# vikshiv/mumemto

Hardware: AMD Instinct MI355X
Metric: input Gbp/s end-to-end (higher is better)
Workload: dtype u8 text, u32 (+u8 beyond 2^32) positions, u32 LCP

## Files before the change

### __graft_entry__.py

```python
import os
import sys

ROOT = os.path.dirname(os.path.abspath(__file__))
for p in (ROOT, os.path.join(ROOT, "oracle")):
    if p not in sys.path:
        sys.path.insert(0, p)


def build():
    import subprocess
    from mumemto_amd import build as mbuild
    lib = mbuild.build(verbose=True)
    assert os.path.exists(lib)
    subprocess.check_call(["make", "-C", os.path.join(ROOT, "oracle"), "all"])
    subprocess.check_call(["make", "-C", os.path.join(ROOT, "tests", "fake_rccl")])
    subprocess.check_call(["make", "-C", os.path.join(ROOT, "tests", "corrupt_rccl")])
    subprocess.check_call(["make", "-C", os.path.join(ROOT, "tests", "kprobe")])
    subprocess.check_call(["make", "-C", os.path.join(ROOT, "tests", "kprobe_input")])
    import mumemto_amd
    mumemto_amd.load_library()


def smoke():
    import numpy as np
    import mumemto_amd
    import pyoracle as O
    from mumemto_amd import synth

    docs = synth.pangenome(6, 50000, 0.01, seed=4, inversion=(2, 10000, 14000))
    eng = mumemto_amd.Engine(0)
    eng.set_docs(docs)
    eng.run(merge_metadata=True)
    want = O.run(docs, merge=True)
# ... 17 lines not shown
```

### mumemto_amd/csrc/engine.hpp

```cpp
#pragma once
#include <cstdint>
#include <cstring>
#include <functional>
#include <memory>
#include <string>
#include <vector>

#include "../../include/mumemto_gpu.h"
#include "device_utils.hpp"
#include "kernels.hpp"
#include "merge_types.hpp"
#include "pfp.hpp"
#include "piece_writer.hpp"
#include "sorter.hpp"
#include "textref.hpp"

namespace mmt {

struct HostRows {
    bool mum_mode = true;
    size_t n_docs = 0, n_rows = 0, n_occ = 0;
    const uint32_t* length = nullptr;
    const int64_t* mum_offsets = nullptr;
    const uint8_t* mum_strands = nullptr;
// ... 172 lines not shown
    void pfp_prepare(uint32_t w, uint32_t p);
    void pfp_prepare_emitter(uint32_t w);
    void pfp_group_tables(uint32_t E, uint32_t G, uint64_t out_lo, uint64_t out_hi, bool slim);
    void pfp_emit_codes(int shift);
    void guided_prepare();
    void guided_check_errors(const char* what);
    void build_giant(const std::vector<uint64_t>& hist);
    static int symbol_codes(const std::vector<uint64_t>& hist, int lowest, bool dollar, uint8_t code[256]);
    struct RunEnds { DevBuf<uint32_t> ends, sorted, count; };
    struct DictLcpScratch { DevBuf<uint32_t> plcp, counts, huge; };
    int sort_dictionary(const uint8_t* dict, uint32_t nd, const std::vector<uint64_t>& hist, DevBuf<uint8_t>& code, uint32_t reserve,
                        int chars_cap, DevBuf<uint32_t>& sa, DevBuf<uint32_t>& rank, RunEnds* run_list);
    void dictionary_lcp(const uint8_t* dict, uint32_t nd, uint32_t* sa, const uint32_t* esuf, const uint8_t* ebw,
                        DevBuf<uint32_t>& lcp, DictLcpScratch& X, uint32_t cap, const char* whose);
    void sort_parse();
    void build_inverted_lists(bool rec12, bool drop_other_form, uint32_t pos_bits, uint32_t* k_in, uint32_t* v_in);
    void pfp_stream(ScanState& S, const mmt_params& p);
    void pfp_emit_window(uint64_t b0, uint64_t c1, int set);
    uint64_t pfp_first_tile(uint64_t b0);
    void guided_stream(ScanState& S, const mmt_params& p);
    void guided_stream_expand(ScanState& S, const mmt_params& p);
    void lcp_bwt();
    void scan(const mmt_params& p);
    void scan_begin(const mmt_params& p, ScanState& S);
    bool scan_window(ScanState& S, const ColWindow& w, const mmt_params& p);
    void scan_end(ScanState& S);
    void window_reserve(int set, uint64_t entries);
    ColWindow window_view(int set, uint64_t base, uint32_t len, uint32_t first) const;
    bool hand_off_window(ScanState& S, int set, const ColWindow& w, const mmt_params& p, bool closing_entry);
    void shard_range(uint32_t index, uint64_t& lo, uint64_t& hi) const;
    struct GuidedShare { std::vector<uint64_t> pre; uint32_t bin_lo = 0, bin_hi = 0; };
// ... 119 lines not shown
```

### mumemto_amd/csrc/pfp.cpp

```cpp
#include <algorithm>
#include <chrono>
#include <cstdio>
#include <cstdlib>
#include <stdexcept>

#include "engine.hpp"
#include "pfp_kernels.hpp"
#include "pool.hpp"
#include "prims.hpp"

namespace mmt {

static void offsets_from_counts(DevBuf<uint8_t>& temp, const uint32_t* counts, PosBuf& out, size_t n, hipStream_t s) {
    if (out.wide()) prims::exclusive_sum_u32_to_u64(temp, counts, out.p64(), n, s);
    else prims::exclusive_sum_u32(temp, counts, out.p32(), n, s);
}


int Engine::symbol_codes(const std::vector<uint64_t>& hist, int lowest, bool dollar, uint8_t code[256]) {
    int sigma = 0;
    for (int c = 0; c < 256; c++) code[c] = (c >= lowest && (hist[c] || (dollar && c == 2))) ? (uint8_t)(++sigma) : 0;
    return sigma;
}

// ... 58 lines not shown
    MMT_HIP(hipStreamSynchronize(st));
}

void Engine::sort_parse() {
    PfpState& S = *pfp_;
    hipStream_t st = stream_;
    const uint32_t m = S.n_phrases;
    S.sa_p.ensure(m); S.isa_p.ensure(m);
    const int pbits = bit_width_u64((uint64_t)S.n_distinct);
    const int pchars = std::max(1, 64 / pbits);
    sorter_.reserve(m);
    pk::pack_keys_u32(S.parse.get(), m, pbits, pchars, sorter_.keys_in(), sorter_.vals_in(), st);
    S.rounds_parse = sorter_.sort(m, pbits * pchars, (uint64_t)pchars, S.sa_p.get(), S.isa_p.get(), d_temp_, st);
}

void Engine::build_inverted_lists(bool rec12, bool drop_other_form, uint32_t pos_bits, uint32_t* k_in, uint32_t* v_in) {
    PfpState& S = *pfp_;
    const bool W = wide_;
    hipStream_t st = stream_;
    const uint32_t m = S.n_phrases, D = S.n_distinct;
    pk::occ_sequence(S.sa_p.get(), S.pid.get(), m, D, k_in, v_in, st);
    prims::sort_pairs_u32_u32(d_temp_, k_in, S.occ_ids.get(), v_in, S.occ_ts.get(), (size_t)m + 1, 0, bit_width_u64((uint64_t)D), st);
    if (rec12) {
        if (drop_other_form) { S.occ.release(); S.occ_sl.release(); }
        S.occ12.ensure(3 * (size_t)m + 4);
        pk::occ_finish12(S.occ_ids.get(), S.occ_ts.get(), S.sa_p.get(), S.pstart.get(), W, m, S.occ_start.get(),
                         S.occ12.get(), S.plcp.sl.get(), st);
    } else {
        if (drop_other_form) S.occ12.release();
        S.occ.ensure(m); S.occ_sl.ensure(m);
        pk::occ_finish(S.occ_ids.get(), S.occ_ts.get(), S.sa_p.get(), S.pstart.get(), m, S.occ_start.get(), S.occ.get(),
                       pos_bits, S.plcp.sl.get(), S.occ_sl.get(), W, st);
    }
    MMT_HIP(hipStreamSynchronize(st));
}

void Engine::pfp_parse(uint32_t w, uint32_t p, bool keep_dict_inputs) {
    PfpState& S = *pfp_;
    const uint64_t n = n_;
    const bool W = wide_;
    const bool slim = (lean_ || wide_) && !keep_dict_inputs;
    if (w < 1 || w > 32 || p < 1) throw std::runtime_error("PFP window must be in [1, 32] and the modulus positive");
    std::vector<uint64_t> hist;
    d2h(hist, d_hist_.get(), 256, stream_);
// ... 178 lines not shown
    const uint32_t m = S.n_phrases, D = S.n_distinct;
    EventPair e5, e6;
    e5.start(st);
    sort_parse();
    if (slim) { MMT_HIP(hipStreamSynchronize(st)); sorter_.release(); S.isa_p.release(); S.parse.release(); }
    S.plcp.build(text_ref(), n + 1 + w, S.sa_p.get(), S.pid.get(), S.pstart.get(), W, m, d_temp_, st);
    e5.stop(st);
    mem_mark(device_, "parse suffix array + LCP");

    e6.start(st);
    const int shift = bit_width_u64((uint64_t)m + 1);
    const uint32_t nd = S.dict_len;
    const uint32_t pos_bits = W ? (uint32_t)bit_width_u64(n + w + 1) : 32u;
    if ((uint32_t)shift + pos_bits > 64)
        throw std::runtime_error("parse rank and text position do not fit one 64-bit occurrence record");
    S.occ_start.ensure((size_t)D + 2); S.occ.ensure(m);
    S.occ_ids.ensure((size_t)m + 1); S.occ_ts.ensure((size_t)m + 1);
    {
        DevBuf<uint32_t> k_own, v_own;
        uint32_t *k_in, *v_in;
        if (slim) { k_own.ensure((size_t)m + 1); v_own.ensure((size_t)m + 1); k_in = k_own.get(); v_in = v_own.get(); }
        else {
            sorter_.u32_a().ensure((size_t)m + 1); sorter_.u32_b().ensure((size_t)m + 1);
            k_in = sorter_.u32_a().get(); v_in = sorter_.u32_b().get();
        }
        build_inverted_lists(false, false, pos_bits, k_in, v_in);
    }
    if (slim) { S.occ_ids.release(); S.occ_ts.release(); S.sa_p.release(); S.pid.release(); S.pstart.release(); }
    S.vscan.ensure(nd); S.ptab.ensure((size_t)D * 16 + 16);
    prims::exclusive_sum_u32(d_temp_, S.vflag.get(), S.vscan.get(), nd, st);
    const uint32_t E = S.n_entries = read_u32(S.vscan.get() + (nd - 1), st) + read_u32(S.vflag.get() + (nd - 1), st);
    pk::phrase_table(S.occ_start.get(), S.plen.get(), S.rep.get(), D, S.ptab.get(), st);
    S.ce_cnt.ensure(E); S.ce_eoff.ensure(E, W); S.ce_first.ensure(E); S.ce_offm1.ensure(E); S.ce_gs.ensure(E);
    S.ce_bwt.ensure(E); S.ce_hl.ensure(E); S.ce_slen.ensure(E);
    if (!S.gscan.get() || !S.segmin.get()) throw std::runtime_error("PFP tables released too early");
    pk::entry_compact(S.esuf.get(), S.ephr.get(), S.ebw.get(), S.gflag.get(), S.gscan.get(), S.vflag.get(), S.vscan.get(),
                      S.segmin.get(), S.ptab.get(), nd, S.ce_cnt.get(), S.ce_first.get(), S.ce_offm1.get(), S.ce_bwt.get(),
                      S.ce_gs.get(), S.ce_hl.get(), S.ce_slen.get(), st);
    offsets_from_counts(d_temp_, S.ce_cnt.get(), S.ce_eoff, E, st);
    {
        const uint64_t total = S.ce_eoff.read(E - 1, st) + read_u32(S.ce_cnt.get() + (E - 1), st);
        if (total != n + 1) throw std::runtime_error("PFP expansion does not cover the text exactly once");
    }
    if (slim) {
        S.esuf.release(); S.ephr.release(); S.ebw.release(); S.gflag.release(); S.vflag.release(); S.vscan.release();
        S.ptab.release(); S.plen.release(); S.segmin.release();
    }
    S.occ12.release(); S.emit_pos_bits = pos_bits; S.emit_w = w;
    pfp_emit_codes(shift);
    pfp_group_tables(E, S.n_groups, 0, n + 1, slim);
    S.emit_launches = 0;
    S.emit_ready = true;
    S.bwt_ready = true;
    e6.stop(st);
    mem_mark(device_, "lists + emitter tables");
    S.ms[5] = e5.ms(); S.ms[6] = e6.ms();
    sort_rounds_ = S.rounds_dict;
}

void Engine::pfp_group_tables(uint32_t E, uint32_t G, uint64_t out_lo, uint64_t out_hi, bool slim) {
    PfpState& S = *pfp_;
    const bool W = wide_;
    hipStream_t st = stream_;
// ... 50 lines not shown
    MMT_HIP(hipStreamSynchronize(st));
    if (slim) S.gscan.release();

    S.tiles = (out_hi + TILE - 1) / TILE;
    S.tile_base = out_lo / TILE;
    pk::EmitArgs& ea = S.ea;
    ea = pk::EmitArgs();
    ea.wide = W;
    ea.segb = S.segb.get(); ea.sege = S.sege.get(); ea.n_groups = G;
    ea.ce_eoff = S.ce_eoff.get(); ea.ce_cnt = S.ce_cnt.get(); ea.ce_first = S.ce_first.get();
    ea.ce_offm1 = S.ce_offm1.get(); ea.ce_bwt = S.ce_bwt.get(); ea.ce_gs = S.ce_gs.get();
    ea.n = n_;
    ea.fb_group = S.fb_group.get(); ea.fb_off = S.fb_off.get(); ea.n_fb = F; ea.fb_base = 0;
    ea.err = S.err.get();
    ea.ghead = S.ghead.get();
    ea.occ = S.occ.get(); ea.occ_sl = S.occ_sl.get(); ea.occ12 = S.occ12.get(); ea.pos_bits = S.emit_pos_bits;
    ea.rmq = S.plcp.view(); ea.w = S.emit_w;
    ea.bwt_code = S.bwt_code.get(); ea.fb_bits = S.fb_bits;
    S.tile_first.ensure((size_t)(S.tiles - S.tile_base) + 4);
    pk::tile_first(S.segb.get(), G, S.tiles, S.tile_first.get(), W, st, S.tile_base);
    MMT_HIP(hipMemsetAsync(S.err.get(), 0, 64, st));
}

void Engine::pfp_emit_codes(int shift) {
    PfpState& S = *pfp_;
    hipStream_t st = stream_;
    S.decode = pk::BwtDecode{};
    S.fb_bits = 0; S.key_shift = shift;
    if (!sw::on(sw::MMT_PFP_NO_BWT_CODE)) {
        std::vector<uint64_t> hist;
        d2h(hist, d_hist_.get(), 256, st);
// ... 164 lines not shown
```

### mumemto_amd/csrc/pfp.hpp

```cpp
#pragma once
#include <unordered_map>
#include <cstdint>
#include <vector>

#include "device_utils.hpp"
#include "parse_lcp.hpp"
#include "guided_kernels.hpp"
#include "pfp_kernels.hpp"

namespace mmt {

struct PfpSummary {
    uint32_t w = 0, p = 0;
    uint32_t n_cuts = 0, n_phrases = 0, n_distinct = 0, dict_len = 0, n_groups = 0;
    bool guided = false;
    bool expand = false;
    int rounds_dict = 0, rounds_parse = 0;
    uint64_t run_refined = 0;
    float ms[8] = {0};
    uint32_t n_entries = 0, n_fallback = 0, emit_launches = 0;
    bool bwt_ready = false;
    int g_prefix = 0;
    uint32_t g_share_lo = 0, g_share_hi = 0;
    int g_bits = 0;
// ... 3 lines not shown

struct PfpState : PfpSummary {
    bool have_parse = false;
    DevBuf<uint8_t> dict, ptab, pinfo;
    DevBuf<uint16_t> tmask;
    DevBuf<uint32_t> tcnt, toff;
    PosBuf cuts, pstart;
    DevBuf<uint32_t> plen, iota, ord_a, order, scan, dflags, pid, rep, dlen, dstart, esuf, ephr;
    DevBuf<uint64_t> dinfo;
    DevBuf<uint8_t> ebw;
    DevBuf<uint32_t> sa_d, rank_d, gflag, pflag, gscan, pscan, prank, parse, sa_p, isa_p, err;
    DevBuf<uint64_t> h1, h2, hk_a, hk_b;
    DevBuf<uint32_t> occ_start, occ_ids, occ_ts, vflag, vscan;
    DevBuf<uint64_t> occ;
    DevBuf<uint32_t> occ12;
    uint32_t emit_pos_bits = 0, emit_w = 0;
    DevBuf<uint32_t> ce_cnt, ce_first, ce_offm1, ce_gs, sege, xk_a, xk_b, fb_group, fb_size, fb_rel, tile_first;
    DevBuf<uint8_t> emit_plan;
    PosBuf ce_eoff, segb, fb_off, fb_start, xv_a, xv_b;
    DevBuf<uint8_t> ce_bwt, bwt_code;
    ParseLcp plcp;
    DevBuf<uint32_t> ghead, ce_hl, ce_slen, occ_sl, lcp_d;
    DevBuf<uint64_t> segmin;
    std::unordered_map<uint64_t, uint64_t> first_tile;
    bool emit_ready = false;
    pk::EmitArgs ea;
    pk::BwtDecode decode{};
    uint32_t fb_bits = 0;
    int key_shift = 0;
    uint64_t tiles = 0, tile_base = 0;
// ... 16 lines not shown
```

### mumemto_amd/csrc/pfp_kernels.hip

```cpp
#include <hip/hip_runtime.h>

#include <algorithm>
#include <cstddef>
#include <cstdint>
#include <cstdlib>
#include <string>

#include "device_utils.hpp"
#include "kernels.hpp"
#include "launch_grid.hpp"
#include "pfp_kernels.hpp"

namespace mmt { namespace pk {

template <int BLOCK>
__global__ __launch_bounds__(BLOCK) void k_trigger_masks(const TextRef T, uint64_t n, uint32_t w,
                                                         uint32_t p, uint32_t pot,
                                                         uint16_t* __restrict__ masks,
                                                         uint32_t* __restrict__ block_count, uint32_t block0) {
    constexpr int PER = 16;
    __shared__ uint32_t s_cnt;
    if (threadIdx.x == 0) s_cnt = 0;
    __syncthreads();
    const uint64_t blk = (uint64_t)blockIdx.x + block0;
// ... 607 lines not shown
__global__ void k_occ_sequence(const uint32_t* __restrict__ sa_p, const uint32_t* __restrict__ pid, uint32_t m,
                               uint32_t D, uint32_t* __restrict__ keys, uint32_t* __restrict__ vals) {
    const uint32_t t = blockIdx.x * blockDim.x + threadIdx.x;
    if (t > m) return;
    uint32_t id;
    if (t == 0) id = pid[m - 1];
    else { const uint32_t q1 = sa_p[t - 1]; id = q1 ? pid[q1 - 1] : D; }
    keys[t] = id;
    vals[t] = t;
}
void occ_sequence(const uint32_t* sa_p, const uint32_t* pid, uint32_t m, uint32_t D, uint32_t* keys, uint32_t* vals,
                  hipStream_t s) {
    hipLaunchKernelGGL(k_occ_sequence, dim3(grid_for((uint64_t)m + 1, 256)), dim3(256), 0, s, sa_p, pid, m, D, keys, vals);
    MMT_HIP(hipGetLastError());
}
template <typename P>
__global__ void k_occ_finish(const uint32_t* __restrict__ ids, const uint32_t* __restrict__ ts,
                             const uint32_t* __restrict__ sa_p, const P* __restrict__ pstart, uint32_t m,
                             uint32_t* __restrict__ occ_start, uint64_t* __restrict__ occ, uint32_t pos_bits,
                             const uint32_t* __restrict__ sl, uint32_t* __restrict__ occ_sl) {
    const uint32_t k = blockIdx.x * blockDim.x + threadIdx.x;
    if (k > m) return;
    const uint32_t id = ids[k];
    if (k == 0 || id != ids[k - 1]) occ_start[id] = k;
    if (k == m) return;
    const uint32_t t = ts[k];
    const uint32_t q = t ? sa_p[t - 1] - 1 : m - 1;
    occ[k] = ((uint64_t)t << pos_bits) | (uint64_t)pstart[q];
    occ_sl[k] = t ? sl[t - 1] : 0u;
}
// ... 1 lines not shown
__global__ void k_occ_finish12(const uint32_t* __restrict__ ids, const uint32_t* __restrict__ ts,
                               const uint32_t* __restrict__ sa_p, const P* __restrict__ pstart, uint32_t m,
                               uint32_t* __restrict__ occ_start, uint32_t* __restrict__ occ12, const uint32_t* __restrict__ sl) {
    const uint32_t k = blockIdx.x * blockDim.x + threadIdx.x;
    if (k > m) return;
    const uint32_t id = ids[k];
    if (k == 0 || id != ids[k - 1]) occ_start[id] = k;
    if (k == m) return;
    const uint32_t t = ts[k];
    const uint32_t q = t ? sa_p[t - 1] - 1 : m - 1;
    const uint64_t pos = (uint64_t)pstart[q];
    const uint32_t v = t ? sl[t - 1] : 0u;
    occ12[3ull * k] = t;
    occ12[3ull * k + 1] = (uint32_t)pos;
    occ12[3ull * k + 2] = ((uint32_t)(pos >> 32) & 0xffu) | ((v < 0xffffffu ? v : 0xffffffu) << 8);
}
void occ_finish12(const uint32_t* ids, const uint32_t* ts, const uint32_t* sa_p, const void* pstart, bool wide, uint32_t m,
                  uint32_t* occ_start, uint32_t* occ12, const uint32_t* sl, hipStream_t s) {
    if (wide)
        hipLaunchKernelGGL(k_occ_finish12<uint64_t>, dim3(grid_for((uint64_t)m + 1, 256)), dim3(256), 0, s, ids, ts, sa_p,
                           static_cast<const uint64_t*>(pstart), m, occ_start, occ12, sl);
    else
        hipLaunchKernelGGL(k_occ_finish12<uint32_t>, dim3(grid_for((uint64_t)m + 1, 256)), dim3(256), 0, s, ids, ts, sa_p,
                           static_cast<const uint32_t*>(pstart), m, occ_start, occ12, sl);
    MMT_HIP(hipGetLastError());
}
void occ_finish(const uint32_t* ids, const uint32_t* ts, const uint32_t* sa_p, const void* pstart, uint32_t m,
                uint32_t* occ_start, uint64_t* occ, uint32_t pos_bits, const uint32_t* sl, uint32_t* occ_sl, bool wide,
                hipStream_t s) {
    if (wide)
// ... 83 lines not shown
        hi = nhi < hi ? nhi : hi;
    }
    const uint32_t i = lo + lane;
    const bool ge = i >= hi ? true : a[i] >= x;
    const uint64_t m = __ballot(ge);
    return m ? lo + (uint32_t)__builtin_ctzll(m) : hi;
}

template <typename P, typename SA>
struct EmitArgsT {
    const P* segb; const uint32_t* sege; uint32_t n_groups;
    const P* ce_eoff; const uint32_t* ce_cnt; const uint32_t* ce_first; const uint32_t* ce_offm1;
    const uint8_t* ce_bwt; const uint32_t* ce_gs;
    const uint64_t* occ; const uint32_t* occ_sl; uint32_t pos_bits;
    const uint32_t* occ12;
    P n;
    SA sa; uint8_t* bwt;
    const uint32_t* fb_group; const P* fb_off; uint32_t n_fb; P fb_base;
    uint32_t* fb_keys; P* fb_vals;
    const uint8_t* bwt_code; uint32_t fb_bits;
    uint32_t* err;
    uint64_t tile_lo;
    uint32_t* lcp; const uint2* ghead; RmqView rmq; uint32_t w;
    uint64_t out_base, win_lo, win_hi;
    uint32_t many_runs;
    uint32_t abl2;
};
template <int BLOCK, int CAP, typename ES = uint32_t>
struct EmitShared {
    alignas(8) uint32_t efirst[CAP];
    uint32_t eoffm1[CAP];
    uint32_t key[CAP];
    ES estart[CAP + 1];
    uint16_t egfirst[CAP];
    uint16_t egs[CAP];
    uint16_t owner[CAP];
    uint8_t ebwt[CAP];
    uint32_t wmax[BLOCK / 64], gwmax[BLOCK / 64];
    uint32_t bound[4];
    uint32_t many;
    uint64_t origin;
};

template <int BLOCK, int CAP, typename P, typename SA, typename ES, int ABL = 0>
__device__ __forceinline__ void emit_piece(const EmitArgsT<P, SA>& a, EmitShared<BLOCK, CAP, ES>& sh, uint32_t e0, uint32_t e1,
                                           P clo, uint32_t L, bool sorted, P fb_origin, uint32_t gbase) {
    using EmitSh = EmitShared<BLOCK, CAP, ES>;
    const uint32_t tid = threadIdx.x, lane = tid & 63, wave = tid >> 6;
    const uint32_t E = e1 - e0;
    const uint64_t pos_mask = (1ull << a.pos_bits) - 1ull;
    __syncthreads();
    for (uint32_t i = tid; i < L; i += BLOCK) sh.owner[i] = 0;
    __syncthreads();
    for (uint32_t e = tid; e < E; e += BLOCK) {
        const uint32_t st = (uint32_t)(a.ce_eoff[e0 + e] - clo);
        sh.estart[e] = (ES)st;
        sh.efirst[e] = a.ce_first[e0 + e];
        sh.eoffm1[e] = a.ce_offm1[e0 + e];
        sh.ebwt[e] = a.ce_bwt[e0 + e];
        const uint32_t gs = a.ce_gs[e0 + e];
        sh.egs[e] = (uint16_t)(gs ? (sorted ? gs - gbase : 1u) : 0u);
        sh.owner[st < L ? st : 0u] = (uint16_t)e;
    }
    if (tid == 0) { sh.estart[E] = (ES)L; sh.many = 0; }
    __syncthreads();
// ... 36 lines not shown
                if (sorted && (i + 1 == E || sh.egs[i + 1]) && i - gf >= a.many_runs) atomicMax(&sh.many, i - gf + 1);
            }
        }
    }
    __syncthreads();
    constexpr int PERX = CAP / BLOCK;
    P my_pos[PERX];
    uint32_t my_sl[PERX];
#pragma unroll
    for (int q = 0; q < PERX; q++) {
        const uint32_t i = tid + q * BLOCK;
        my_sl[q] = 0;
        if (i < L) {
            const uint32_t e = sh.owner[i], k = i - sh.estart[e];
            uint32_t key;
            if (a.occ12 && ABL != 3) {
                const uint32_t* r = a.occ12 + 3ull * ((uint64_t)sh.efirst[e] + k);
                const uint32_t r0 = r[0], r1 = r[1], r2 = r[2];
                key = r0;
                my_pos[q] = (P)(((uint64_t)r1 | ((uint64_t)(r2 & 0xffu) << 32)) + sh.eoffm1[e]);
                if (sorted) { const uint32_t v = r2 >> 8; my_sl[q] = v == 0xffffffu && r0 ? a.rmq.sl[r0 - 1] : v; }
            } else {
                const uint64_t kp = ABL == 3 ? ((uint64_t)(i + 1) << a.pos_bits) | 7u : a.occ[sh.efirst[e] + k];
                if (sorted && ABL != 3) my_sl[q] = a.occ_sl[sh.efirst[e] + k];
                key = (uint32_t)(kp >> a.pos_bits);
                my_pos[q] = (P)((kp & pos_mask) + sh.eoffm1[e]);
            }
            if (sorted) sh.key[i] = key;
            else {
                const uint32_t slot = (uint32_t)(clo - fb_origin) + i;
                a.fb_keys[slot] = a.fb_bits ? (key << a.fb_bits) | a.bwt_code[sh.ebwt[e]] : key;
                a.fb_vals[slot] = my_pos[q];
            }
        }
    }
    if (!sorted) return;
    __syncthreads();
    uint2 g_head[PERX];
    uint32_t my_e[PERX], my_gf[PERX], my_gs[PERX];
#pragma unroll
    for (int q = 0; q < PERX; q++) {
// ... 233 lines not shown
    uint8_t ebwt[CAP];
    uint32_t omask[CAP / 32];
    uint32_t gmask[CAP / 32 + 1];
    uint32_t bound[4];
    uint32_t many;
};

template <int BLOCK, int CAP, typename P, typename SA>
__device__ __forceinline__ void emit_tile_piece(const EmitArgsT<P, SA>& a, EmitTile<BLOCK, CAP>& sh, uint32_t e0, uint32_t e1,
                                                P clo, uint32_t L) {
    using Sh = EmitTile<BLOCK, CAP>;
    constexpr int PER = CAP / BLOCK;
    constexpr uint32_t MW = CAP / 32;
    const uint32_t tid = threadIdx.x;
    const uint32_t E = e1 - e0;
    const uint64_t pos_mask = (1ull << a.pos_bits) - 1ull;
    __syncthreads();
    for (uint32_t e = tid; e < E; e += BLOCK) {
        const uint32_t st = (uint32_t)(a.ce_eoff[e0 + e] - clo);
        const uint32_t gs = a.ce_gs[e0 + e];
        const uint32_t fi = a.ce_first[e0 + e], om = a.ce_offm1[e0 + e];
        const uint8_t bw = a.ce_bwt[e0 + e];
        sh.estart[e] = (uint16_t)st;
        sh.efirst[e] = fi;
        sh.eoffm1[e] = om;
        sh.ebwt[e] = bw;
        if (st < (uint32_t)CAP) {
            sh.owner_at[st] = (uint16_t)e;
            atomicOr(&sh.omask[st >> 5], 1u << (st & 31));
        }
        if (gs) { atomicOr(&sh.gmask[e >> 5], 1u << (e & 31)); sh.mpos[e] = gs; }
// ... 13 lines not shown
            uint32_t m = sh.omask[wd] & (0xffffffffu >> (31u - (i & 31u)));
            while (!m && wd) m = sh.omask[--wd];
            const uint32_t p = m ? (wd << 5) + 31u - (uint32_t)__clz(m) : 0u;
            const uint32_t e = sh.owner_at[p], k = i - p;
            wd = e >> 5;
            m = sh.gmask[wd] & (0xffffffffu >> (31u - (e & 31u)));
            while (!m && wd) m = sh.gmask[--wd];
            const uint32_t gf = m ? (wd << 5) + 31u - (uint32_t)__clz(m) : 0u;
            wd = e >> 5;
            m = sh.gmask[wd] & ~(0xffffffffu >> (31u - (e & 31u)));
            while (!m && wd < MW) m = sh.gmask[++wd];
            const uint32_t ge = m ? (wd << 5) + (uint32_t)__ffs(m) - 1u : E;
            const uint32_t fi = sh.efirst[e], om = sh.eoffm1[e];
            uint32_t key;
            if (a.abl2 & 2u) { key = i + 1; my_pos[q] = (P)7; my_sl[q] = 5; }
            else if (a.occ12) {
                const uint32_t* r = a.occ12 + 3ull * ((uint64_t)fi + k);
                const uint32_t r0 = r[0], r1 = r[1], r2 = r[2];
                key = r0;
                my_pos[q] = (P)(((uint64_t)r1 | ((uint64_t)(r2 & 0xffu) << 32)) + om);
                const uint32_t v = r2 >> 8;
                my_sl[q] = v == 0xffffffu && r0 ? a.rmq.sl[r0 - 1] : v;
            } else {
                const uint64_t kp = a.occ[fi + k];
                my_sl[q] = a.occ_sl[fi + k];
                key = (uint32_t)(kp >> a.pos_bits);
                my_pos[q] = (P)((kp & pos_mask) + om);
            }
            if (!(a.abl2 & 8u)) g_head[q] = a.ghead[sh.mpos[gf] - 1u];
            my_gs[q] = sh.estart[gf];
            my_run[q] = e | (gf << 10) | (ge << 20);
            sh.key[i] = key;
            if (ge - gf - 1u >= a.many_runs) any_many = true;
        }
    }
    if (any_many) sh.many = 1u;
    __syncthreads();
    if (tid < MW) sh.omask[tid] = 0u;
    if (tid <= MW) sh.gmask[tid] = 0u;
    uint32_t my_slot[PER];
    if (sh.many) {
        uint64_t* const sk = reinterpret_cast<uint64_t*>(sh.efirst);
// ... 63 lines not shown
        if (i < L) {
            const uint32_t slot = my_slot[q];
            const uint64_t pos = (uint64_t)my_pos[q];
            merged[slot] = make_uint2(sh.key[i], my_sl[q]);
            sh.mpos[slot] = (uint32_t)pos;
            mhb[slot] = (uint16_t)(((uint32_t)(pos >> 32) & 0xffu) | ((uint32_t)sh.ebwt[my_run[q] & 1023u] << 8));
        }
    }
    __syncthreads();
    uint32_t t_lo[PER], t_hi[PER], mn0[PER], sl_first[PER];
#pragma unroll
    for (int q = 0; q < PER; q++) {
        const uint32_t i = tid + q * BLOCK;
        t_lo[q] = 0; t_hi[q] = 0; mn0[q] = 0; sl_first[q] = 0xffffffffu;
        if (i < L && i != my_gs[q]) {
            const uint2 cur = merged[i];
            t_lo[q] = merged[i - 1].x; t_hi[q] = cur.x; mn0[q] = cur.y;
            if (t_lo[q] != 0 && t_hi[q] > t_lo[q] + 1u && !(a.abl2 & 1u)) sl_first[q] = a.rmq.sl[t_lo[q]];
        }
    }
#pragma unroll
    for (int q = 0; q < PER; q++) {
        const uint32_t i = tid + q * BLOCK;
        if (i < L) {
            const uint64_t out = (uint64_t)clo + i;
            const uint32_t hb = mhb[i];
            const uint64_t pos = (uint64_t)sh.mpos[i] | ((uint64_t)(hb & 0xffu) << 32);
            if (out == 0) {
                if (pos != (uint64_t)a.n) { atomicAdd(a.err, 1u); atomicAdd(a.err + 4, 1u); }
                continue;
            }
            if (pos >= (uint64_t)a.n) {
                atomicAdd(a.err, 1u);
// ... 76 lines not shown
        if (t_next >= n_tiles) break;
        t = t_next; d = dn;
    }
}

uint32_t emit_tile() {
    const int v = sw::num(sw::MMT_EMIT_TILE, 896);
    return (uint32_t)(v == 1024 || v == 768 ? v : 896);
}
template <typename P, typename SA, int TILE, int BLOCK = 256>
static void emit_typed(const EmitArgs& a, const uint32_t* tile_first_tab, uint64_t tile_base, void* plan, uint64_t tile_lo, uint64_t tile_hi, hipStream_t s) {
    constexpr int CAP = (int)EMIT_CAP;
    EmitArgsT<P, SA> t;
    t.segb = static_cast<const P*>(a.segb); t.sege = a.sege; t.n_groups = a.n_groups;
    t.ce_eoff = static_cast<const P*>(a.ce_eoff); t.ce_cnt = a.ce_cnt; t.ce_first = a.ce_first; t.ce_offm1 = a.ce_offm1;
    t.ce_bwt = a.ce_bwt; t.ce_gs = a.ce_gs; t.occ = a.occ; t.occ_sl = a.occ_sl; t.pos_bits = a.pos_bits; t.occ12 = a.occ12; t.n = (P)a.n;
    t.sa = SA(a.sa); t.bwt = a.bwt;
    t.fb_group = a.fb_group; t.fb_off = static_cast<const P*>(a.fb_off); t.n_fb = a.n_fb; t.fb_base = (P)a.fb_base;
    t.fb_keys = a.fb_keys; t.fb_vals = static_cast<P*>(a.fb_vals);
    t.bwt_code = a.bwt_code; t.fb_bits = a.fb_bits; t.err = a.err; t.tile_lo = tile_lo;
    t.lcp = a.lcp; t.ghead = static_cast<const uint2*>(a.ghead); t.rmq = a.rmq; t.w = a.w;
    t.out_base = a.out_base; t.win_lo = a.win_lo; t.win_hi = a.win_hi;
    t.many_runs = (uint32_t)sw::num(sw::MMT_EMIT_MANY, 24);
    t.abl2 = (uint32_t)sw::num(sw::MMT_EMIT2_ABLATE, 0);
    const uint32_t n_tiles = (uint32_t)(tile_hi - tile_lo);
    EmitDesc* desc = static_cast<EmitDesc*>(plan);
    hipLaunchKernelGGL((k_emit_plan<P, TILE, CAP>), dim3(grid_for(n_tiles, 256)), dim3(256), 0, s, t.segb, t.sege, tile_first_tab,
                       tile_base, tile_lo, n_tiles, desc);
    const uint32_t grid_env = (uint32_t)sw::num(sw::MMT_EMIT_GRID, 256 * 7 * 4);
    const uint32_t grid = grid_env ? std::min(grid_env, n_tiles) : n_tiles;
    const int abl = sw::num(sw::MMT_EMIT_ABLATE, 0);
// ... 46 lines not shown
        const uint32_t first = wave_lower_bound<P>(a.ce_eoff + e_lo, e_hi - e_lo, (P)(X0 + 1));
        const uint32_t end = wave_lower_bound<P>(a.ce_eoff + e_lo, e_hi - e_lo, (P)(X0 + L));
        if (lane == 0) { sh.bound[1] = e_lo + first - 1; sh.bound[2] = e_lo + end; }
    }
    __syncthreads();
    const uint32_t e0 = sh.bound[1], e1 = sh.bound[2];
    emit_piece<BLOCK, CAP, P, SA, uint32_t>(a, sh, e0, e1, (P)X0, L, false, fb_origin, 0u);
}
template <typename P, typename SA>
static void emit_big_typed(const EmitArgs& a, const uint64_t* chunk0, uint32_t f0, uint32_t nf, uint32_t n_chunks, hipStream_t s) {
    constexpr int BLOCK = 256, CAP = (int)EMIT_CAP;
    static_assert(EMIT_BIG_CHUNK + 1 <= EMIT_CAP, "a chunk's entries (one per element + the one that began before it) must fit the tile tables");
    EmitArgsT<P, SA> t;
    t.segb = static_cast<const P*>(a.segb); t.sege = a.sege; t.n_groups = a.n_groups;
    t.ce_eoff = static_cast<const P*>(a.ce_eoff); t.ce_cnt = a.ce_cnt; t.ce_first = a.ce_first; t.ce_offm1 = a.ce_offm1;
    t.ce_bwt = a.ce_bwt; t.ce_gs = a.ce_gs; t.occ = a.occ; t.occ_sl = a.occ_sl; t.pos_bits = a.pos_bits; t.occ12 = a.occ12; t.n = (P)a.n;
    t.sa = SA(a.sa); t.bwt = a.bwt;
    t.fb_group = a.fb_group; t.fb_off = static_cast<const P*>(a.fb_off); t.n_fb = a.n_fb; t.fb_base = (P)a.fb_base;
    t.fb_keys = a.fb_keys; t.fb_vals = static_cast<P*>(a.fb_vals);
    t.bwt_code = a.bwt_code; t.fb_bits = a.fb_bits; t.err = a.err; t.tile_lo = 0;
    t.lcp = a.lcp; t.ghead = static_cast<const uint2*>(a.ghead); t.rmq = a.rmq; t.w = a.w;
    t.out_base = a.out_base; t.win_lo = a.win_lo; t.win_hi = a.win_hi; t.many_runs = 0xffffffffu; t.abl2 = 0;
    hipLaunchKernelGGL((k_emit_big<BLOCK, CAP, P, SA>), dim3(n_chunks), dim3(BLOCK), 0, s, t, chunk0, f0, nf);
    MMT_HIP(hipGetLastError());
}
void emit_big(const EmitArgs& a, const uint64_t* chunk0, uint32_t f0, uint32_t nf, uint64_t n_chunks, hipStream_t s) {
    if (!nf || !n_chunks) return;
    if (n_chunks > 0x7fffffffull) throw std::runtime_error("too many chunks of oversized suffix groups in one emitter launch");
    if (a.wide) emit_big_typed<uint64_t, Sa40>(a, chunk0, f0, nf, (uint32_t)n_chunks, s);
    else emit_big_typed<uint32_t, Sa32>(a, chunk0, f0, nf, (uint32_t)n_chunks, s);
}
// ... 137 lines not shown
```

### mumemto_amd/csrc/pfp_kernels.hpp

```cpp
#pragma once
#include <cstdint>

#include <hip/hip_runtime_api.h>

#include "parse_lcp.hpp"
#include "textref.hpp"
#include "wide.hpp"

namespace mmt { namespace pk {

constexpr uint32_t KR_PRIME = 1999999973u;
inline uint64_t kr_window_of_run(uint8_t c, uint32_t w) {
    uint64_t h = 0;
    for (uint32_t i = 0; i < w; i++) h = (h * 256 + c) % KR_PRIME;
    return h;
}

uint32_t trigger_blocks(uint64_t n);
void trigger_masks(const TextRef& text, uint64_t n, uint32_t w, uint32_t p, uint16_t* masks, uint32_t* block_count,
                   hipStream_t s);
void trigger_cuts(const uint16_t* masks, uint64_t n, const uint32_t* block_off, void* cuts, bool wide, hipStream_t s);
void phrase_bounds(const void* cuts, uint32_t n_cuts, uint64_t n, uint32_t w, void* start, uint32_t* len, bool wide,
                   hipStream_t s);
void phrase_hash(const TextRef& v, const void* start, const uint32_t* len, uint32_t m, uint64_t* h1, void* pinfo,
// ... 13 lines not shown
                      uint32_t* plcp, void* longs, uint32_t* long_count, uint32_t long_cap, hipStream_t s);
void dict_lcp_clamp(uint32_t* lcp, const uint32_t* esuf, uint32_t nd, hipStream_t s);
void group_flags(const uint32_t* esuf, const uint32_t* lcp_d, uint32_t nd, uint32_t w, uint32_t* gflag, uint32_t* pflag,
                 uint32_t* vflag, uint64_t* seg, hipStream_t s);
void phrase_ranks(const uint32_t* esuf, const uint32_t* ephr, const uint32_t* pscan, uint32_t nd, uint32_t* prank,
                  hipStream_t s);
void phrase_table(const uint32_t* occ_start , const uint32_t* plen, const uint32_t* rep,
                  uint32_t n_distinct, void* tab, hipStream_t s);
void occ_sequence(const uint32_t* sa_p, const uint32_t* pid, uint32_t m, uint32_t D, uint32_t* keys, uint32_t* vals,
                  hipStream_t s);
void occ_finish(const uint32_t* ids, const uint32_t* ts, const uint32_t* sa_p, const void* pstart, uint32_t m,
                uint32_t* occ_start, uint64_t* occ, uint32_t pos_bits, const uint32_t* sl, uint32_t* occ_sl, bool wide,
                hipStream_t s);
void occ_finish12(const uint32_t* ids, const uint32_t* ts, const uint32_t* sa_p, const void* pstart, bool wide, uint32_t m,
                  uint32_t* occ_start, uint32_t* occ12, const uint32_t* sl, hipStream_t s);
void entry_compact(const uint32_t* esuf, const uint32_t* ephr, const uint8_t* ebw, const uint32_t* gflag,
                   const uint32_t* gscan, const uint32_t* vflag, const uint32_t* vscan, const uint64_t* segmin,
                   const void* tab, uint32_t nd, uint32_t* ce_cnt, uint32_t* ce_first, uint32_t* ce_offm1,
                   uint8_t* ce_bwt, uint32_t* ce_gs, uint32_t* ce_hl, uint32_t* ce_slen, hipStream_t s);
void group_heads(const uint32_t* sege, const uint32_t* ce_hl, const uint32_t* ce_slen, uint32_t n_groups, void* ghead,
                 hipStream_t s);
void parse_ranks(const uint32_t* pid, const uint32_t* prank, uint32_t m, uint32_t* parse, hipStream_t s);
void invert_ranks(const uint32_t* prank, const uint32_t* rep, const uint32_t* dlen, uint32_t n_distinct,
                  uint32_t* which, uint32_t* slen, hipStream_t s);
void pack_keys_u32(const uint32_t* parse, uint32_t m, int bits, int chars, uint64_t* keys, uint32_t* vals,
                   hipStream_t s);
static const uint32_t EMIT_CAP = 1024;
uint32_t emit_tile();
struct EmitArgs {
    bool wide;
    const void* segb;
    const uint32_t* sege;
    uint32_t n_groups;
    const void* ce_eoff; const uint32_t* ce_cnt; const uint32_t* ce_first; const uint32_t* ce_offm1;
    const uint8_t* ce_bwt; const uint32_t* ce_gs;
    const uint64_t* occ;
    const uint32_t* occ_sl = nullptr;
    const uint32_t* occ12 = nullptr;
    uint32_t pos_bits;
    uint64_t n;
    SaCol sa; uint8_t* bwt;
    const uint32_t* fb_group; const void* fb_off; uint32_t n_fb;
    uint64_t fb_base;
    uint32_t* fb_keys; void* fb_vals;
    const uint8_t* bwt_code; uint32_t fb_bits;
    uint32_t* err;
    uint32_t* lcp = nullptr;
    const void* ghead = nullptr;
    RmqView rmq;
    uint32_t w = 0;
    uint64_t out_base = 0, win_lo = 0, win_hi = ~0ull;
};
struct BwtDecode { uint8_t byte[16]; };
// ... 17 lines not shown
```

Baseline: 3.843.

## Pack occurrence records with both neighbouring phrase LCPs into joined 12-byte layout

Adds a joined occurrence record format (occj) holding the packed rank/position plus 16-bit clamped LCP values for both the preceding and following parse suffix. The emit kernels read this through a common accessor, and the grouped-merge path pulls the neighbour LCPs from the merged record instead of gathering from the RMQ sl array, falling back to a global read only when the value saturates. This is meant to cut scattered global reads of sl during emission, at the cost of a 12-byte record instead of 8+4 and a saturation fallback path.

```diff
diff --git a/__graft_entry__.py b/__graft_entry__.py
--- a/__graft_entry__.py
+++ b/__graft_entry__.py
@@ -17,6 +17,7 @@
     subprocess.check_call(["make", "-C", os.path.join(ROOT, "tests", "corrupt_rccl")])
     subprocess.check_call(["make", "-C", os.path.join(ROOT, "tests", "kprobe")])
     subprocess.check_call(["make", "-C", os.path.join(ROOT, "tests", "kprobe_input")])
+    subprocess.check_call(["make", "-C", os.path.join(ROOT, "tests", "kprobe_occ")])
     import mumemto_amd
     mumemto_amd.load_library()
 
diff --git a/mumemto_amd/csrc/engine.hpp b/mumemto_amd/csrc/engine.hpp
--- a/mumemto_amd/csrc/engine.hpp
+++ b/mumemto_amd/csrc/engine.hpp
@@ -210,7 +210,7 @@
     void dictionary_lcp(const uint8_t* dict, uint32_t nd, uint32_t* sa, const uint32_t* esuf, const uint8_t* ebw,
                         DevBuf<uint32_t>& lcp, DictLcpScratch& X, uint32_t cap, const char* whose);
     void sort_parse();
-    void build_inverted_lists(bool rec12, bool drop_other_form, uint32_t pos_bits, uint32_t* k_in, uint32_t* v_in);
+    void build_inverted_lists(bool rec12, bool drop_other_form, uint32_t pos_bits, uint32_t* k_in, uint32_t* v_in, bool joined = false);
     void pfp_stream(ScanState& S, const mmt_params& p);
     void pfp_emit_window(uint64_t b0, uint64_t c1, int set);
     uint64_t pfp_first_tile(uint64_t b0);
diff --git a/mumemto_amd/csrc/pfp.cpp b/mumemto_amd/csrc/pfp.cpp
--- a/mumemto_amd/csrc/pfp.cpp
+++ b/mumemto_amd/csrc/pfp.cpp
@@ -96,20 +96,24 @@
     S.rounds_parse = sorter_.sort(m, pbits * pchars, (uint64_t)pchars, S.sa_p.get(), S.isa_p.get(), d_temp_, st);
 }
 
-void Engine::build_inverted_lists(bool rec12, bool drop_other_form, uint32_t pos_bits, uint32_t* k_in, uint32_t* v_in) {
+void Engine::build_inverted_lists(bool rec12, bool drop_other_form, uint32_t pos_bits, uint32_t* k_in, uint32_t* v_in, bool joined) {
     PfpState& S = *pfp_;
     const bool W = wide_;
     hipStream_t st = stream_;
     const uint32_t m = S.n_phrases, D = S.n_distinct;
     pk::occ_sequence(S.sa_p.get(), S.pid.get(), m, D, k_in, v_in, st);
     prims::sort_pairs_u32_u32(d_temp_, k_in, S.occ_ids.get(), v_in, S.occ_ts.get(), (size_t)m + 1, 0, bit_width_u64((uint64_t)D), st);
-    if (rec12) {
-        if (drop_other_form) { S.occ.release(); S.occ_sl.release(); }
+    if (joined) {
+        S.occj.ensure(3 * (size_t)m + 4);
+        pk::occ_finish_joined(S.occ_ids.get(), S.occ_ts.get(), S.sa_p.get(), S.pstart.get(), W, m, S.occ_start.get(),
+                              S.occj.get(), pos_bits, S.plcp.sl.get(), st);
+    } else if (rec12) {
+        if (drop_other_form) { S.occ.release(); S.occ_sl.release(); S.occj.release(); }
         S.occ12.ensure(3 * (size_t)m + 4);
         pk::occ_finish12(S.occ_ids.get(), S.occ_ts.get(), S.sa_p.get(), S.pstart.get(), W, m, S.occ_start.get(),
                          S.occ12.get(), S.plcp.sl.get(), st);
     } else {
-        if (drop_other_form) S.occ12.release();
+        if (drop_other_form) { S.occ12.release(); S.occj.release(); }
         S.occ.ensure(m); S.occ_sl.ensure(m);
         pk::occ_finish(S.occ_ids.get(), S.occ_ts.get(), S.sa_p.get(), S.pstart.get(), m, S.occ_start.get(), S.occ.get(),
                        pos_bits, S.plcp.sl.get(), S.occ_sl.get(), W, st);
@@ -318,7 +322,7 @@
     const uint32_t pos_bits = W ? (uint32_t)bit_width_u64(n + w + 1) : 32u;
     if ((uint32_t)shift + pos_bits > 64)
         throw std::runtime_error("parse rank and text position do not fit one 64-bit occurrence record");
-    S.occ_start.ensure((size_t)D + 2); S.occ.ensure(m);
+    S.occ_start.ensure((size_t)D + 2); S.occj.ensure(3 * (size_t)m + 4);
     S.occ_ids.ensure((size_t)m + 1); S.occ_ts.ensure((size_t)m + 1);
     {
         DevBuf<uint32_t> k_own, v_own;
@@ -328,7 +332,7 @@
             sorter_.u32_a().ensure((size_t)m + 1); sorter_.u32_b().ensure((size_t)m + 1);
             k_in = sorter_.u32_a().get(); v_in = sorter_.u32_b().get();
         }
-        build_inverted_lists(false, false, pos_bits, k_in, v_in);
+        build_inverted_lists(false, false, pos_bits, k_in, v_in, true);
     }
     if (slim) { S.occ_ids.release(); S.occ_ts.release(); S.sa_p.release(); S.pid.release(); S.pstart.release(); }
     S.vscan.ensure(nd); S.ptab.ensure((size_t)D * 16 + 16);
@@ -350,7 +354,7 @@
         S.esuf.release(); S.ephr.release(); S.ebw.release(); S.gflag.release(); S.vflag.release(); S.vscan.release();
         S.ptab.release(); S.plen.release(); S.segmin.release();
     }
-    S.occ12.release(); S.emit_pos_bits = pos_bits; S.emit_w = w;
+    S.occ12.release(); S.occ.release(); S.occ_sl.release(); S.emit_pos_bits = pos_bits; S.emit_w = w;
     pfp_emit_codes(shift);
     pfp_group_tables(E, S.n_groups, 0, n + 1, slim);
     S.emit_launches = 0;
@@ -431,7 +435,7 @@
     ea.fb_group = S.fb_group.get(); ea.fb_off = S.fb_off.get(); ea.n_fb = F; ea.fb_base = 0;
     ea.err = S.err.get();
     ea.ghead = S.ghead.get();
-    ea.occ = S.occ.get(); ea.occ_sl = S.occ_sl.get(); ea.occ12 = S.occ12.get(); ea.pos_bits = S.emit_pos_bits;
+    ea.occ = S.occ.get(); ea.occ_sl = S.occ_sl.get(); ea.occ12 = S.occ12.get(); ea.occj = S.occj.get(); ea.pos_bits = S.emit_pos_bits;
     ea.rmq = S.plcp.view(); ea.w = S.emit_w;
     ea.bwt_code = S.bwt_code.get(); ea.fb_bits = S.fb_bits;
     S.tile_first.ensure((size_t)(S.tiles - S.tile_base) + 4);
diff --git a/mumemto_amd/csrc/pfp.hpp b/mumemto_amd/csrc/pfp.hpp
--- a/mumemto_amd/csrc/pfp.hpp
+++ b/mumemto_amd/csrc/pfp.hpp
@@ -41,6 +41,7 @@
     DevBuf<uint32_t> occ_start, occ_ids, occ_ts, vflag, vscan;
     DevBuf<uint64_t> occ;
     DevBuf<uint32_t> occ12;
+    DevBuf<uint32_t> occj;
     uint32_t emit_pos_bits = 0, emit_w = 0;
     DevBuf<uint32_t> ce_cnt, ce_first, ce_offm1, ce_gs, sege, xk_a, xk_b, fb_group, fb_size, fb_rel, tile_first;
     DevBuf<uint8_t> emit_plan;
diff --git a/mumemto_amd/csrc/pfp_kernels.hip b/mumemto_amd/csrc/pfp_kernels.hip
--- a/mumemto_amd/csrc/pfp_kernels.hip
+++ b/mumemto_amd/csrc/pfp_kernels.hip
@@ -645,6 +645,7 @@
     hipLaunchKernelGGL(k_occ_sequence, dim3(grid_for((uint64_t)m + 1, 256)), dim3(256), 0, s, sa_p, pid, m, D, keys, vals);
     MMT_HIP(hipGetLastError());
 }
+constexpr uint32_t OCC_ASK = 0xffffu;
 template <typename P>
 __global__ void k_occ_finish(const uint32_t* __restrict__ ids, const uint32_t* __restrict__ ts,
                              const uint32_t* __restrict__ sa_p, const P* __restrict__ pstart, uint32_t m,
@@ -676,6 +677,34 @@
     occ12[3ull * k] = t;
     occ12[3ull * k + 1] = (uint32_t)pos;
     occ12[3ull * k + 2] = ((uint32_t)(pos >> 32) & 0xffu) | ((v < 0xffffffu ? v : 0xffffffu) << 8);
+}
+template <typename P>
+__global__ void k_occ_finish_joined(const uint32_t* __restrict__ ids, const uint32_t* __restrict__ ts,
+                                    const uint32_t* __restrict__ sa_p, const P* __restrict__ pstart, uint32_t m,
+                                    uint32_t* __restrict__ occ_start, uint32_t* __restrict__ occj, uint32_t pos_bits,
+                                    const uint32_t* __restrict__ sl) {
+    const uint32_t k = blockIdx.x * blockDim.x + threadIdx.x;
+    if (k > m) return;
+    const uint32_t id = ids[k];
+    if (k == 0 || id != ids[k - 1]) occ_start[id] = k;
+    if (k == m) return;
+    const uint32_t t = ts[k];
+    const uint32_t q = t ? sa_p[t - 1] - 1 : m - 1;
+    const uint32_t before = t ? sl[t - 1] : 0u, behind = t < m ? sl[t] : OCC_ASK;
+    const uint64_t rec = ((uint64_t)t << pos_bits) | (uint64_t)pstart[q];
+    occj[3ull * k] = (uint32_t)rec;
+    occj[3ull * k + 1] = (uint32_t)(rec >> 32);
+    occj[3ull * k + 2] = (before < OCC_ASK ? before : OCC_ASK) | ((behind < OCC_ASK ? behind : OCC_ASK) << 16);
+}
+void occ_finish_joined(const uint32_t* ids, const uint32_t* ts, const uint32_t* sa_p, const void* pstart, bool wide, uint32_t m,
+                       uint32_t* occ_start, uint32_t* occj, uint32_t pos_bits, const uint32_t* sl, hipStream_t s) {
+    if (wide)
+        hipLaunchKernelGGL(k_occ_finish_joined<uint64_t>, dim3(grid_for((uint64_t)m + 1, 256)), dim3(256), 0, s, ids, ts, sa_p,
+                           static_cast<const uint64_t*>(pstart), m, occ_start, occj, pos_bits, sl);
+    else
+        hipLaunchKernelGGL(k_occ_finish_joined<uint32_t>, dim3(grid_for((uint64_t)m + 1, 256)), dim3(256), 0, s, ids, ts, sa_p,
+                           static_cast<const uint32_t*>(pstart), m, occ_start, occj, pos_bits, sl);
+    MMT_HIP(hipGetLastError());
 }
 void occ_finish12(const uint32_t* ids, const uint32_t* ts, const uint32_t* sa_p, const void* pstart, bool wide, uint32_t m,
                   uint32_t* occ_start, uint32_t* occ12, const uint32_t* sl, hipStream_t s) {
@@ -789,6 +818,7 @@
     const uint8_t* ce_bwt; const uint32_t* ce_gs;
     const uint64_t* occ; const uint32_t* occ_sl; uint32_t pos_bits;
     const uint32_t* occ12;
+    const uint32_t* occj;
     P n;
     SA sa; uint8_t* bwt;
     const uint32_t* fb_group; const P* fb_off; uint32_t n_fb; P fb_base;
@@ -817,13 +847,36 @@
     uint64_t origin;
 };
 
+struct OccRec { uint32_t t; uint64_t pos; uint32_t prev, next; };
+template <typename P, typename SA>
+__device__ __forceinline__ OccRec occ_record(const EmitArgsT<P, SA>& a, uint64_t k) {
+    OccRec o;
+    if (a.occj) {
+        const uint32_t* r = a.occj + 3ull * k;
+        const uint32_t r0 = r[0], r1 = r[1], r2 = r[2];
+        const uint64_t kp = (uint64_t)r0 | ((uint64_t)r1 << 32);
+        o.t = (uint32_t)(kp >> a.pos_bits); o.pos = kp & ((1ull << a.pos_bits) - 1ull);
+        o.prev = r2 & 0xffffu; o.next = r2 >> 16;
+    } else if (a.occ12) {
+        const uint32_t* r = a.occ12 + 3ull * k;
+        const uint32_t r0 = r[0], r1 = r[1], r2 = r[2];
+        o.t = r0; o.pos = (uint64_t)r1 | ((uint64_t)(r2 & 0xffu) << 32);
+        o.prev = (r2 >> 8) < OCC_ASK ? r2 >> 8 : OCC_ASK; o.next = OCC_ASK;
+    } else {
+        const uint64_t kp = a.occ[k];
+        const uint32_t v = a.occ_sl[k];
+        o.t = (uint32_t)(kp >> a.pos_bits); o.pos = kp & ((1ull << a.pos_bits) - 1ull);
+        o.prev = v < OCC_ASK ? v : OCC_ASK; o.next = OCC_ASK;
+    }
+    return o;
+}
+
 template <int BLOCK, int CAP, typename P, typename SA, typename ES, int ABL = 0>
 __device__ __forceinline__ void emit_piece(const EmitArgsT<P, SA>& a, EmitShared<BLOCK, CAP, ES>& sh, uint32_t e0, uint32_t e1,
                                            P clo, uint32_t L, bool sorted, P fb_origin, uint32_t gbase) {
     using EmitSh = EmitShared<BLOCK, CAP, ES>;
     const uint32_t tid = threadIdx.x, lane = tid & 63, wave = tid >> 6;
     const uint32_t E = e1 - e0;
-    const uint64_t pos_mask = (1ull << a.pos_bits) - 1ull;
     __syncthreads();
     for (uint32_t i = tid; i < L; i += BLOCK) sh.owner[i] = 0;
     __syncthreads();
@@ -890,17 +943,12 @@
         if (i < L) {
             const uint32_t e = sh.owner[i], k = i - sh.estart[e];
             uint32_t key;
-            if (a.occ12 && ABL != 3) {
-                const uint32_t* r = a.occ12 + 3ull * ((uint64_t)sh.efirst[e] + k);
-                const uint32_t r0 = r[0], r1 = r[1], r2 = r[2];
-                key = r0;
-                my_pos[q] = (P)(((uint64_t)r1 | ((uint64_t)(r2 & 0xffu) << 32)) + sh.eoffm1[e]);
-                if (sorted) { const uint32_t v = r2 >> 8; my_sl[q] = v == 0xffffffu && r0 ? a.rmq.sl[r0 - 1] : v; }
-            } else {
-                const uint64_t kp = ABL == 3 ? ((uint64_t)(i + 1) << a.pos_bits) | 7u : a.occ[sh.efirst[e] + k];
-                if (sorted && ABL != 3) my_sl[q] = a.occ_sl[sh.efirst[e] + k];
-                key = (uint32_t)(kp >> a.pos_bits);
-                my_pos[q] = (P)((kp & pos_mask) + sh.eoffm1[e]);
+            if (ABL == 3) { key = i + 1; my_pos[q] = (P)(7u + sh.eoffm1[e]); }
+            else {
+                const OccRec o = occ_record(a, (uint64_t)sh.efirst[e] + k);
+                key = o.t;
+                my_pos[q] = (P)(o.pos + sh.eoffm1[e]);
+                if (sorted) my_sl[q] = o.prev == OCC_ASK && o.t ? a.rmq.sl[o.t - 1] : o.prev;
             }
             if (sorted) sh.key[i] = key;
             else {
@@ -1164,7 +1212,6 @@
     constexpr uint32_t MW = CAP / 32;
     const uint32_t tid = threadIdx.x;
     const uint32_t E = e1 - e0;
-    const uint64_t pos_mask = (1ull << a.pos_bits) - 1ull;
     __syncthreads();
     for (uint32_t e = tid; e < E; e += BLOCK) {
         const uint32_t st = (uint32_t)(a.ce_eoff[e0 + e] - clo);
@@ -1208,18 +1255,11 @@
             const uint32_t fi = sh.efirst[e], om = sh.eoffm1[e];
             uint32_t key;
             if (a.abl2 & 2u) { key = i + 1; my_pos[q] = (P)7; my_sl[q] = 5; }
-            else if (a.occ12) {
-                const uint32_t* r = a.occ12 + 3ull * ((uint64_t)fi + k);
-                const uint32_t r0 = r[0], r1 = r[1], r2 = r[2];
-                key = r0;
-                my_pos[q] = (P)(((uint64_t)r1 | ((uint64_t)(r2 & 0xffu) << 32)) + om);
-                const uint32_t v = r2 >> 8;
-                my_sl[q] = v == 0xffffffu && r0 ? a.rmq.sl[r0 - 1] : v;
-            } else {
-                const uint64_t kp = a.occ[fi + k];
-                my_sl[q] = a.occ_sl[fi + k];
-                key = (uint32_t)(kp >> a.pos_bits);
-                my_pos[q] = (P)((kp & pos_mask) + om);
+            else {
+                const OccRec o = occ_record(a, (uint64_t)fi + k);
+                key = o.t;
+                my_pos[q] = (P)(o.pos + om);
+                my_sl[q] = o.prev | (o.next << 16);
             }
             if (!(a.abl2 & 8u)) g_head[q] = a.ghead[sh.mpos[gf] - 1u];
             my_gs[q] = sh.estart[gf];
@@ -1313,9 +1353,13 @@
         const uint32_t i = tid + q * BLOCK;
         t_lo[q] = 0; t_hi[q] = 0; mn0[q] = 0; sl_first[q] = 0xffffffffu;
         if (i < L && i != my_gs[q]) {
-            const uint2 cur = merged[i];
-            t_lo[q] = merged[i - 1].x; t_hi[q] = cur.x; mn0[q] = cur.y;
-            if (t_lo[q] != 0 && t_hi[q] > t_lo[q] + 1u && !(a.abl2 & 1u)) sl_first[q] = a.rmq.sl[t_lo[q]];
+            const uint2 cur = merged[i], low = merged[i - 1];
+            t_lo[q] = low.x; t_hi[q] = cur.x; mn0[q] = cur.y & 0xffffu;
+            if (mn0[q] == OCC_ASK && t_hi[q] != 0) mn0[q] = a.rmq.sl[t_hi[q] - 1u];
+            if (t_lo[q] != 0 && t_hi[q] > t_lo[q] + 1u && !(a.abl2 & 1u)) {
+                sl_first[q] = low.y >> 16;
+                if (sl_first[q] == OCC_ASK) sl_first[q] = a.rmq.sl[t_lo[q]];
+            }
         }
     }
 #pragma unroll
@@ -1422,7 +1466,7 @@
     EmitArgsT<P, SA> t;
     t.segb = static_cast<const P*>(a.segb); t.sege = a.sege; t.n_groups = a.n_groups;
     t.ce_eoff = static_cast<const P*>(a.ce_eoff); t.ce_cnt = a.ce_cnt; t.ce_first = a.ce_first; t.ce_offm1 = a.ce_offm1;
-    t.ce_bwt = a.ce_bwt; t.ce_gs = a.ce_gs; t.occ = a.occ; t.occ_sl = a.occ_sl; t.pos_bits = a.pos_bits; t.occ12 = a.occ12; t.n = (P)a.n;
+    t.ce_bwt = a.ce_bwt; t.ce_gs = a.ce_gs; t.occ = a.occ; t.occ_sl = a.occ_sl; t.pos_bits = a.pos_bits; t.occ12 = a.occ12; t.occj = a.occj; t.n = (P)a.n;
     t.sa = SA(a.sa); t.bwt = a.bwt;
     t.fb_group = a.fb_group; t.fb_off = static_cast<const P*>(a.fb_off); t.n_fb = a.n_fb; t.fb_base = (P)a.fb_base;
     t.fb_keys = a.fb_keys; t.fb_vals = static_cast<P*>(a.fb_vals);
@@ -1499,7 +1543,7 @@
     EmitArgsT<P, SA> t;
     t.segb = static_cast<const P*>(a.segb); t.sege = a.sege; t.n_groups = a.n_groups;
     t.ce_eoff = static_cast<const P*>(a.ce_eoff); t.ce_cnt = a.ce_cnt; t.ce_first = a.ce_first; t.ce_offm1 = a.ce_offm1;
-    t.ce_bwt = a.ce_bwt; t.ce_gs = a.ce_gs; t.occ = a.occ; t.occ_sl = a.occ_sl; t.pos_bits = a.pos_bits; t.occ12 = a.occ12; t.n = (P)a.n;
+    t.ce_bwt = a.ce_bwt; t.ce_gs = a.ce_gs; t.occ = a.occ; t.occ_sl = a.occ_sl; t.pos_bits = a.pos_bits; t.occ12 = a.occ12; t.occj = a.occj; t.n = (P)a.n;
     t.sa = SA(a.sa); t.bwt = a.bwt;
     t.fb_group = a.fb_group; t.fb_off = static_cast<const P*>(a.fb_off); t.n_fb = a.n_fb; t.fb_base = (P)a.fb_base;
     t.fb_keys = a.fb_keys; t.fb_vals = static_cast<P*>(a.fb_vals);
diff --git a/mumemto_amd/csrc/pfp_kernels.hpp b/mumemto_amd/csrc/pfp_kernels.hpp
--- a/mumemto_amd/csrc/pfp_kernels.hpp
+++ b/mumemto_amd/csrc/pfp_kernels.hpp
@@ -51,6 +51,8 @@
                 hipStream_t s);
 void occ_finish12(const uint32_t* ids, const uint32_t* ts, const uint32_t* sa_p, const void* pstart, bool wide, uint32_t m,
                   uint32_t* occ_start, uint32_t* occ12, const uint32_t* sl, hipStream_t s);
+void occ_finish_joined(const uint32_t* ids, const uint32_t* ts, const uint32_t* sa_p, const void* pstart, bool wide, uint32_t m,
+                       uint32_t* occ_start, uint32_t* occj, uint32_t pos_bits, const uint32_t* sl, hipStream_t s);
 void entry_compact(const uint32_t* esuf, const uint32_t* ephr, const uint8_t* ebw, const uint32_t* gflag,
                    const uint32_t* gscan, const uint32_t* vflag, const uint32_t* vscan, const uint64_t* segmin,
                    const void* tab, uint32_t nd, uint32_t* ce_cnt, uint32_t* ce_first, uint32_t* ce_offm1,
@@ -74,6 +76,7 @@
     const uint64_t* occ;
     const uint32_t* occ_sl = nullptr;
     const uint32_t* occ12 = nullptr;
+    const uint32_t* occj = nullptr;
     uint32_t pos_bits;
     uint64_t n;
     SaCol sa; uint8_t* bwt;
```

Result: slower. 3.723 (-3.1%).
